# google/automl

Measured on NVIDIA H100. Metric: EfficientDet-D0 images/sec @ batch 32/GPU (640x640, forward + post-process), higher is better.
Workload: dtype f16 storage / f32 accumulate

## Files before the change

automl_b200/csrc/pointwise_tc.cu:

```cuda
#include <math_constants.h>

#include <type_traits>

#include "tc_common.cuh"

namespace edet {
namespace pwtc {

constexpr int BLOCK_M = 64;
constexpr int kMaxBlockN = 128;
template <int TEAMS>
struct Epi {
  static constexpr int kThreads = 128 * (1 + TEAMS);
};
constexpr int kStoreCols = 64;
constexpr int kSlabBytes = BLOCK_M * kStoreCols * 2;
constexpr int kMaxStages = 9;
constexpr int kRing = 4;
constexpr int kSmemLimit = 227 * 1024;
constexpr int kResidentWBytes = 108 * 1024;

struct Params {
  int batch, rows, k, nout, nout_pad8;
  int block_n, num_m_blocks, num_n_blocks, num_k_blocks, num_stages;
  int team_stages;
  int block_k;
  int a_stage_bytes, b_stage_bytes;
  int stage_bytes;
  int w_resident;
  int slab_sets;
  int slab_set_bytes;
  int desc_sbo;
  int desc_layout;
  int wbatch, ldr;
  int total_tiles;
  int bias_floats;
  const float* bias;
  const __half* residual;
  unsigned* sched;
  float* am_scores;
  int32_t* am_classes;
  int am_anchor_begin, am_total, am_num_anchors;
};
constexpr int EPI_STORE = 0, EPI_ARGMAX = 1;
constexpr int kArgmaxCols = 96;

struct TileCoord {
  int b, m_blk, n_blk;
};
constexpr int kMaxBiasSmem = 8192;

__device__ __forceinline__ TileCoord decode_tile(int t, const Params& p) {
  TileCoord c;
  c.n_blk = 0;
  if (p.num_n_blocks != 1) {
    c.n_blk = t % p.num_n_blocks;
    t /= p.num_n_blocks;
  }
  c.m_blk = t;
  c.b = 0;
  if (p.batch != 1) {
    c.m_blk = t % p.num_m_blocks;
    c.b = t / p.num_m_blocks;
  }
  return c;
}

__device__ __forceinline__ uint32_t argmax_pair_key(float2 s, uint32_t col) {
  const __half2 h = __hadd2(__floats2half2_rn(s.x, s.y), __float2half2_rn(0.f));
  const uint32_t hb = *reinterpret_cast<const uint32_t*>(&h);
  uint32_t sgn;
  asm("prmt.b32 %0, %1, %2, 0xBB99;" : "=r"(sgn) : "r"(hb), "r"(0u));
  const uint32_t ord = hb ^ (sgn | 0x80008000u);
  const uint32_t codes = ((0xFFFFu - (col + 1u)) << 16) | (0xFFFFu - col);
  uint32_t k0, k1;
  asm("prmt.b32 %0, %1, %2, 0x1054;" : "=r"(k0) : "r"(ord), "r"(codes));
  asm("prmt.b32 %0, %1, %2, 0x3276;" : "=r"(k1) : "r"(ord), "r"(codes));
  return max(k0, k1);
}

template <int ACT, bool HAS_RES, int TEAMS, int EPI>
__global__ void __launch_bounds__(Epi<TEAMS>::kThreads, 1)
pointwise_tc_kernel(const __grid_constant__ CUtensorMap map_a,
                    const __grid_constant__ CUtensorMap map_w,
                    const __grid_constant__ CUtensorMap map_o, const Params p) {
  pdl_launch_dependents();
  extern __shared__ __align__(1024) uint8_t smem_raw[];
  uint8_t* smem = reinterpret_cast<uint8_t*>(
      (reinterpret_cast<uintptr_t>(smem_raw) + 1023) & ~static_cast<uintptr_t>(1023));
  const int stage_bytes = p.stage_bytes;
  uint8_t* smem_w = smem + p.num_stages * stage_bytes;
  const int w_bytes = p.w_resident ? p.num_n_blocks * p.num_k_blocks * p.b_stage_bytes : 0;
  uint8_t* smem_store = smem_w + w_bytes;
  float* smem_bias = reinterpret_cast<float*>(smem_store + TEAMS * p.slab_sets * p.slab_set_bytes);
  uint64_t* bars = reinterpret_cast<uint64_t*>(smem_bias + p.bias_floats);
  uint64_t* full_bar = bars;
  uint64_t* empty_bar = bars + kMaxStages;
  uint64_t* ring_full = bars + 2 * kMaxStages;
  uint64_t* ring_empty = ring_full + kRing;
  uint64_t* w_full = ring_empty + kRing;
  volatile int4* tile_ring = reinterpret_cast<volatile int4*>(w_full + 2);

  const int warp = __shfl_sync(0xffffffffu, static_cast<int>(threadIdx.x >> 5), 0);
  const int lane = threadIdx.x & 31;

  if (threadIdx.x == 0) {
    for (int s = 0; s < p.num_stages; ++s) {
      mbar_init(smem_u32(&full_bar[s]), 1);
      mbar_init(smem_u32(&empty_bar[s]), 4);
    }
    for (int s = 0; s < kRing; ++s) {
      mbar_init(smem_u32(&ring_full[s]), 1);
      mbar_init(smem_u32(&ring_empty[s]), TEAMS);
    }
    mbar_init(smem_u32(&w_full[0]), 1);
    asm volatile("fence.mbarrier_init.release.cluster;" ::: "memory");
    asm volatile("prefetch.tensormap [%0];" ::"l"(reinterpret_cast<uint64_t>(&map_a)) : "memory");
    asm volatile("prefetch.tensormap [%0];" ::"l"(reinterpret_cast<uint64_t>(&map_w)) : "memory");
    asm volatile("prefetch.tensormap [%0];" ::"l"(reinterpret_cast<uint64_t>(&map_o)) : "memory");
  }
  for (int i = threadIdx.x; i < p.bias_floats; i += blockDim.x)
    smem_bias[i] = i < p.nout ? __ldg(p.bias + i) : 0.f;
  __syncthreads();
  pdl_wait_prior();

  if (warp == 0) {
    if (lane == 0) {
      const uint32_t w_box_bytes = static_cast<uint32_t>(p.block_n * p.block_k * 2);
      if (p.w_resident) {
        const uint32_t wb = smem_u32(&w_full[0]);
        mbar_expect_tx(wb, w_box_bytes * p.num_n_blocks * p.num_k_blocks);
        for (int nb = 0; nb < p.num_n_blocks; ++nb)
          for (int kb = 0; kb < p.num_k_blocks; ++kb)
            tma_load_3d(smem_u32(smem_w + (nb * p.num_k_blocks + kb) * p.b_stage_bytes), &map_w,
                        wb, kb * p.block_k, nb * p.block_n, 0);
      }
      int stage_of[TEAMS] = {}, phase_of[TEAMS] = {};
      const uint32_t tx_bytes =
          static_cast<uint32_t>(p.a_stage_bytes) + (p.w_resident ? 0u : w_box_bytes);
      bool exhausted = false;
      for (int i = 0;; ++i) {
        int t = p.total_tiles;
        if (i == 0) {
          t = blockIdx.x;
        } else if (!exhausted) {
          t = sched_next_tile(p.sched, p.total_tiles);
          exhausted = t >= p.total_tiles;
        }
        const int slot = i & (kRing - 1);
        mbar_wait(smem_u32(&ring_empty[slot]), (static_cast<uint32_t>(i / kRing) & 1u) ^ 1u);
        TileCoord tc;
        tc.b = tc.m_blk = tc.n_blk = 0;
        if (t < p.total_tiles) tc = decode_tile(t, p);
        const_cast<int4*>(tile_ring)[slot] = make_int4(t, tc.b, tc.m_blk, tc.n_blk);
        mbar_arrive(smem_u32(&ring_full[slot]));
        if (t >= p.total_tiles) break;
        const int wb = (p.wbatch > 1) ? tc.b : 0;
        const int team = i % TEAMS;
        int stage = stage_of[team];
        uint32_t phase = static_cast<uint32_t>(phase_of[team]);
        for (int kb = 0; kb < p.num_k_blocks; ++kb) {
          const int s = team * p.team_stages + stage;
          mbar_wait(smem_u32(&empty_bar[s]), phase ^ 1);
          const uint32_t fb = smem_u32(&full_bar[s]);
          mbar_expect_tx(fb, tx_bytes);
          uint8_t* sa = smem + s * stage_bytes;
          tma_load_3d(smem_u32(sa), &map_a, fb, kb * p.block_k, tc.m_blk * BLOCK_M, tc.b);
          if (!p.w_resident)
            tma_load_3d(smem_u32(sa + p.a_stage_bytes), &map_w, fb, kb * p.block_k,
                        tc.n_blk * p.block_n, wb);
          if (++stage == p.team_stages) {
            stage = 0;
            phase ^= 1;
          }
        }
        stage_of[team] = stage;
        phase_of[team] = static_cast<int>(phase);
      }
    }
  } else if (warp >= 4) {
    const int team = (warp >> 2) - 1;
    const int wtid = threadIdx.x & 127;
    const int r0 = 16 * (warp & 3) + (lane >> 2);
    const int cq = 2 * (lane & 3);
    uint8_t* team_slabs = smem_store + team * p.slab_sets * p.slab_set_bytes;
    if (p.w_resident) mbar_wait(smem_u32(&w_full[0]), 0);
    auto consume = [&](auto nt_const) {
    constexpr int NT = decltype(nt_const)::value;
    int my_tiles = 0;
    int stage = 0;
    uint32_t phase = 0;
    auto advance = [&]() {
      if (++stage == p.team_stages) {
        stage = 0;
        phase ^= 1;
      }
    };
    for (int iter = 0;; ++iter) {
      const int slot = iter & (kRing - 1);
      mbar_wait(smem_u32(&ring_full[slot]), static_cast<uint32_t>(iter / kRing) & 1u);
      int4 e = const_cast<const int4*>(tile_ring)[slot];
      e.x = __shfl_sync(0xffffffffu, e.x, 0);
      e.y = __shfl_sync(0xffffffffu, e.y, 0);
      e.z = __shfl_sync(0xffffffffu, e.z, 0);
      e.w = __shfl_sync(0xffffffffu, e.w, 0);
      named_sync(1 + team, 128);
      if (wtid == 0) mbar_arrive(smem_u32(&ring_empty[slot]));
      const int t = e.x;
      if (t >= p.total_tiles) break;
      if (iter % TEAMS != team) continue;
      TileCoord tc;
      tc.b = e.y;
      tc.m_blk = e.z;
      tc.n_blk = e.w;
      const int n0 = tc.n_blk * p.block_n;
      const int n_valid = min(p.block_n, ((p.nout - n0 + 15) >> 4) << 4);
      const int nt = n_valid >> 4;
      float acc[NT][8];
#pragma unroll
      for (int j = 0; j < NT; ++j)
#pragma unroll
        for (int q = 0; q < 8; ++q) acc[j][q] = 0.f;
      int prev_s = -1;
      for (int kb = 0; kb < p.num_k_blocks; ++kb) {
        const int s = team * p.team_stages + stage;
        mbar_wait(smem_u32(&full_bar[s]), phase);
        uint8_t* sa = smem + s * stage_bytes;
        uint8_t* sb = p.w_resident
                          ? smem_w + (tc.n_blk * p.num_k_blocks + kb) * p.b_stage_bytes
                          : sa + p.a_stage_bytes;
        const uint64_t da = make_smem_desc(smem_u32(sa), p.desc_sbo, p.desc_layout);
        const uint64_t db = make_smem_desc(smem_u32(sb), p.desc_sbo, p.desc_layout);
        const int k_rem = p.k - kb * p.block_k;
        const int ksteps = k_rem >= p.block_k ? p.block_k / MMA_K : (k_rem + MMA_K - 1) / MMA_K;
        wg_fence();
        wg_mma_kblock_wide<NT>(acc, da, db, ksteps, kb == 0);
        wg_commit();
        wg_wait<1>();
        if (prev_s >= 0) {
          __syncwarp();
          if (lane == 0) mbar_arrive(smem_u32(&empty_bar[prev_s]));
        }
        prev_s = s;
        advance();
      }
      wg_wait<0>();
      __syncwarp();
      if (lane == 0) mbar_arrive(smem_u32(&empty_bar[prev_s]));
      wg_fence_acc<NT>(acc);
      const int row0 = tc.m_blk * BLOCK_M + r0;
      if constexpr (EPI == EPI_ARGMAX) {
        const float* bias = smem_bias + tc.n_blk * kArgmaxCols;
        uint32_t best[2] = {0u, 0u};
#pragma unroll
        for (int j = 0; j < kArgmaxCols / 16; ++j) {
#pragma unroll
          for (int h = 0; h < 2; ++h) {
            const int col = 16 * j + 8 * h + cq;
            const float2 b = *reinterpret_cast<const float2*>(bias + col);
#pragma unroll
            for (int r = 0; r < 2; ++r) {
              const float2 s = fadd2_rn(make_float2(acc[j][4 * h + 2 * r], acc[j][4 * h + 2 * r + 1]), b);
              best[r] = max(best[r], argmax_pair_key(s, static_cast<uint32_t>(col)));
            }
          }
        }
#pragma unroll
        for (int r = 0; r < 2; ++r) {
          best[r] = max(best[r], __shfl_xor_sync(0xffffffffu, best[r], 1));
          best[r] = max(best[r], __shfl_xor_sync(0xffffffffu, best[r], 2));
          const uint32_t ord_best = best[r] >> 16;
          const unsigned short hbits = static_cast<unsigned short>(
              (ord_best & 0x8000u) ? (ord_best ^ 0x8000u) : (~ord_best & 0xFFFFu));
          const float bv = __half2float(__ushort_as_half(hbits));
          const int best_c = static_cast<int>(0xFFFFu - (best[r] & 0xFFFFu));
          const int row = row0 + 8 * r;
          if ((lane & 3) == 0 && row < p.rows) {
            const size_t o = static_cast<size_t>(tc.b) * p.am_total + p.am_anchor_begin +
                             static_cast<size_t>(row) * p.am_num_anchors + tc.n_blk;
            p.am_scores[o] = __fdiv_rn(1.0f, __fadd_rn(1.0f, expf(-bv)));
            p.am_classes[o] = best_c;
          }
        }
      } else {
        const bool ok[2] = {row0 < p.rows, row0 + 8 < p.rows};
        const __half* res_row[2] = {nullptr, nullptr};
        if (HAS_RES) {
#pragma unroll
          for (int r = 0; r < 2; ++r)
            res_row[r] = p.residual +
                         (static_cast<size_t>(tc.b) * p.rows + (ok[r] ? row0 + 8 * r : 0)) * p.ldr;
        }
        uint8_t* my_slabs = team_slabs + (my_tiles % p.slab_sets) * p.slab_set_bytes;
        ++my_tiles;
        if (wtid == 0) {
          if (p.slab_sets == 2)
            tma_store_wait_read<1>();
          else
            tma_store_wait_read<0>();
        }
        named_sync(1 + team, 128);
#pragma unroll
        for (int j = 0; j < NT; ++j) {
          if (j < nt) {
            const int colt = 16 * j + cq;
            const float2 b_lo = *reinterpret_cast<const float2*>(smem_bias + n0 + colt);
            const float2 b_hi = *reinterpret_cast<const float2*>(smem_bias + n0 + colt + 8);
            uint8_t* slab = my_slabs + (colt >> 6) * kSlabBytes;
            const int piece = (colt & 63) >> 3;
#pragma unroll
            for (int r = 0; r < 2; ++r) {
              float2 lo = fadd2_rn(make_float2(acc[j][2 * r], acc[j][2 * r + 1]), b_lo);
              float2 hi = fadd2_rn(make_float2(acc[j][4 + 2 * r], acc[j][4 + 2 * r + 1]), b_hi);
              apply_act4<ACT>(lo, hi);
              if (HAS_RES && ok[r]) {
                const int col = n0 + colt;
                if (col < p.nout)
                  lo = fadd2_rn(lo, __half22float2(*reinterpret_cast<const __half2*>(res_row[r] + col)));
                if (col + 8 < p.nout)
                  hi = fadd2_rn(hi, __half22float2(*reinterpret_cast<const __half2*>(res_row[r] + col + 8)));
              }
              const int row = r0 + 8 * r;
              uint8_t* rb = slab + row * 128 + cq * 2;
              *reinterpret_cast<__half2*>(rb + ((piece ^ (row & 7)) << 4)) = __floats2half2_rn(lo.x, lo.y);
              *reinterpret_cast<__half2*>(rb + (((piece + 1) ^ (row & 7)) << 4)) = __floats2half2_rn(hi.x, hi.y);
            }
          }
        }
        fence_proxy_async_smem();
        named_sync(1 + team, 128);
        if (wtid == 0) {
          for (int c = 0; c * kStoreCols < n_valid; ++c)
            tma_store_3d(&map_o, smem_u32(my_slabs + c * kSlabBytes), n0 + c * kStoreCols,
                         tc.m_blk * BLOCK_M, tc.b);
          tma_store_commit();
        }
      }
    }
    };
    if constexpr (EPI == EPI_ARGMAX) {
      consume(std::integral_constant<int, kArgmaxCols / 16>{});
    } else {
      switch (p.block_n >> 5) {
        case 1: consume(std::integral_constant<int, 2>{}); break;
        case 2: consume(std::integral_constant<int, 4>{}); break;
        case 3: consume(std::integral_constant<int, 6>{}); break;
        default: consume(std::integral_constant<int, 8>{}); break;
      }
    }
    if (wtid == 0) tma_store_wait_all();
  }
}

static int pick_block_n(int nout) {
  if (nout <= kMaxBlockN) return ((nout + 31) / 32) * 32;
  return kMaxBlockN;
}

template <int ACT, bool HAS_RES, int TEAMS, int EPI = EPI_STORE>
static int launch(const CUtensorMap& ma, const CUtensorMap& mw, const CUtensorMap& mo,
                  const Params& p, int grid, int smem_bytes, cudaStream_t stream) {
  auto kern = pointwise_tc_kernel<ACT, HAS_RES, TEAMS, EPI>;
  static int configured[kMaxDevices];
  if (int rc = ensure_dynamic_smem(kern, kSmemLimit, configured)) return rc;
  EDET_CHECK_CUDA(launch_pdl(kern, dim3(grid), dim3(Epi<TEAMS>::kThreads), smem_bytes, stream, ma,
                             mw, mo, p));
  return EDET_OK;
}

int run(const __half* a, int lda, const __half* wt, int wbatch, const float* bias,
        const __half* residual, int ldr, __half* out, int ldo, int batch, int rows, int k, int nout,
        int act, cudaStream_t stream, const ArgmaxArgs* am) {
  Params p;
  p.am_scores = nullptr; p.am_classes = nullptr;
  p.am_anchor_begin = p.am_total = p.am_num_anchors = 0;
  if (am) {
    EDET_CHECK_ARG(nout == am->num_anchors * kArgmaxCols && !residual && act == EDET_ACT_NONE,
                   "class_argmax: nout must be num_anchors * %d", kArgmaxCols);
    p.am_scores = am->scores; p.am_classes = am->classes;
    p.am_anchor_begin = am->anchor_begin; p.am_total = am->total_anchors;
    p.am_num_anchors = am->num_anchors;
  }
  p.batch = batch;
  p.rows = rows;
  p.k = k;
  p.nout = nout;
  p.nout_pad8 = nout & ~7;
  const int opt_teams = option_pw_teams();
  const int teams = opt_teams ? opt_teams : 2;
  p.block_n = am ? kArgmaxCols : pick_block_n(nout);
  p.num_m_blocks = ceil_div(rows, BLOCK_M);
  p.num_n_blocks = ceil_div(nout, p.block_n);
  p.wbatch = wbatch;
  p.ldr = ldr;
  p.bias = bias;
  p.residual = residual;
  p.total_tiles = batch * p.num_m_blocks * p.num_n_blocks;
  p.sched = next_sched_slot();
  if (!p.sched) return EDET_ERR_CUDA;

  const int bias_cols = p.num_n_blocks * p.block_n;
  EDET_CHECK_ARG(bias_cols <= kMaxBiasSmem, "pointwise_tc: nout %d too wide", nout);
  p.bias_floats = bias_cols;
  p.block_k = k <= 16 ? 16 : (k <= 32 ? 32 : 64);
  p.a_stage_bytes = BLOCK_M * p.block_k * 2;
  p.b_stage_bytes = ((p.block_n * p.block_k * 2 + 1023) / 1024) * 1024;
  p.num_k_blocks = ceil_div(k, p.block_k);
  const int w_bytes = p.num_n_blocks * p.num_k_blocks * p.b_stage_bytes;
  p.w_resident = wbatch == 1 && w_bytes <= kResidentWBytes;
  p.stage_bytes = p.a_stage_bytes + (p.w_resident ? 0 : p.b_stage_bytes);
  p.slab_set_bytes = am ? 0 : ceil_div(p.block_n, kStoreCols) * kSlabBytes;
  const int opt_kb = option_pw_smem_kb();
  const int limit = opt_kb ? opt_kb * 1024 : kSmemLimit;
  auto fixed_bytes = [&](int sets) {
    return (p.w_resident ? w_bytes : 0) + teams * sets * p.slab_set_bytes + p.bias_floats * 4 +
           (2 * kMaxStages + 2 * kRing + 2) * 8 + 16 * kRing;
  };
  p.slab_sets = (limit - 1024 - fixed_bytes(2)) / p.stage_bytes >= 3 * teams ? 2 : 1;
  const int fixed = fixed_bytes(p.slab_sets);
  int stages = (limit - 1024 - fixed) / p.stage_bytes;
  if (stages > kMaxStages) stages = kMaxStages;
  p.team_stages = stages / teams;
  EDET_CHECK_ARG(p.team_stages >= 2, "pointwise_tc: block_n %d leaves <2 pipeline stages per consumer",
                 p.block_n);
  stages = p.team_stages * teams;
  p.num_stages = stages;
  p.desc_layout = desc_layout_for(p.block_k);
  p.desc_sbo = 8 * p.block_k * 2;
  const int smem_bytes = 1024 + stages * p.stage_bytes + fixed;

  CUtensorMap ma, mw, mo;
  int rc;
  if ((rc = make_map(&ma, a, k, rows, batch, lda, static_cast<uint64_t>(rows) * lda, BLOCK_M,
                     p.block_k)))
    return rc;
  if ((rc = make_map(&mw, wt, k, nout, wbatch, k, static_cast<uint64_t>(nout) * k, p.block_n,
                     p.block_k)))
    return rc;
  if (am) {
    mo = mw;
  } else if ((rc = make_map(&mo, out, nout, rows, batch, ldo, static_cast<uint64_t>(rows) * ldo,
                            BLOCK_M, kStoreCols))) {
    return rc;
  }

  const int sm_count = device_sm_count();
  if (!sm_count) return EDET_ERR_CUDA;
  int grid = sm_count - option_persist_slack();
  if (grid < 1) grid = 1;
  if (p.total_tiles < grid) grid = p.total_tiles;
  const bool has_res = residual != nullptr;
  if (am) return launch<EDET_ACT_NONE, false, 2, EPI_ARGMAX>(ma, mw, mo, p, grid, smem_bytes, stream);

#define EDET_PW_CASE(A)                                                                       \
  if (teams == 3)                                                                             \
    return has_res ? launch<A, true, 3>(ma, mw, mo, p, grid, smem_bytes, stream)              \
                   : launch<A, false, 3>(ma, mw, mo, p, grid, smem_bytes, stream);            \
  return has_res ? launch<A, true, 2>(ma, mw, mo, p, grid, smem_bytes, stream)                \
                 : launch<A, false, 2>(ma, mw, mo, p, grid, smem_bytes, stream)
  switch (act) {
    case EDET_ACT_NONE: EDET_PW_CASE(EDET_ACT_NONE);
    case EDET_ACT_SWISH: EDET_PW_CASE(EDET_ACT_SWISH);
    case EDET_ACT_RELU: EDET_PW_CASE(EDET_ACT_RELU);
    case EDET_ACT_RELU6: EDET_PW_CASE(EDET_ACT_RELU6);
    case EDET_ACT_HSWISH: EDET_PW_CASE(EDET_ACT_HSWISH);
    case EDET_ACT_SIGMOID: EDET_PW_CASE(EDET_ACT_SIGMOID);
    default:
      set_error("pointwise_tc: bad activation %d", act);
      return EDET_ERR_INVALID;
  }
#undef EDET_PW_CASE
}

}
}
```

automl_b200/csrc/tc_common.cuh:

```cuda
#pragma once
#include <cuda.h>

#include "common.cuh"

namespace edet {
namespace pwtc {

constexpr int MMA_K = 16;

struct ArgmaxArgs {
  float* scores;
  int32_t* classes;
  int anchor_begin, total_anchors, num_anchors;
};
int run(const __half* a, int lda, const __half* wt, int wbatch, const float* bias,
        const __half* residual, int ldr, __half* out, int ldo, int batch, int rows, int k, int nout,
        int act, cudaStream_t stream, const ArgmaxArgs* am = nullptr);

__device__ __forceinline__ uint32_t smem_u32(const void* p) {
  return static_cast<uint32_t>(__cvta_generic_to_shared(p));
}
__device__ __forceinline__ void mbar_init(uint32_t bar, uint32_t count) {
  asm volatile("mbarrier.init.shared::cta.b64 [%0], %1;" ::"r"(bar), "r"(count));
}
__device__ __forceinline__ void mbar_expect_tx(uint32_t bar, uint32_t bytes) {
  asm volatile("mbarrier.arrive.expect_tx.shared::cta.b64 _, [%0], %1;" ::"r"(bar), "r"(bytes)
               : "memory");
}
__device__ __forceinline__ void mbar_arrive(uint32_t bar) {
  asm volatile("mbarrier.arrive.shared::cta.b64 _, [%0];" ::"r"(bar) : "memory");
}
__device__ __forceinline__ void mbar_wait(uint32_t bar, uint32_t parity) {
  asm volatile(
      "{\n\t"
      ".reg .pred p;\n\t"
      "WAIT_LOOP:\n\t"
      "mbarrier.try_wait.parity.shared::cta.b64 p, [%0], %1;\n\t"
      "@p bra DONE;\n\t"
      "bra WAIT_LOOP;\n\t"
      "DONE:\n\t"
      "}" ::"r"(bar),
      "r"(parity)
      : "memory");
}
__device__ __forceinline__ void tma_load_3d(uint32_t dst, const CUtensorMap* map, uint32_t bar,
                                            int c0, int c1, int c2) {
  asm volatile(
      "cp.async.bulk.tensor.3d.shared::cluster.global.mbarrier::complete_tx::bytes "
      "[%0], [%1, {%3, %4, %5}], [%2];" ::"r"(dst),
      "l"(reinterpret_cast<uint64_t>(map)), "r"(bar), "r"(c0), "r"(c1), "r"(c2)
      : "memory");
}
__device__ __forceinline__ void tma_store_3d(const CUtensorMap* map, uint32_t src, int c0, int c1,
                                             int c2) {
  asm volatile(
      "cp.async.bulk.tensor.3d.global.shared::cta.bulk_group [%0, {%2, %3, %4}], [%1];" ::"l"(
          reinterpret_cast<uint64_t>(map)),
      "r"(src), "r"(c0), "r"(c1), "r"(c2)
      : "memory");
}
__device__ __forceinline__ void tma_store_4d(const CUtensorMap* map, uint32_t src, int c0, int c1,
                                             int c2, int c3) {
  asm volatile(
      "cp.async.bulk.tensor.4d.global.shared::cta.bulk_group [%0, {%2, %3, %4, %5}], [%1];" ::"l"(
          reinterpret_cast<uint64_t>(map)),
      "r"(src), "r"(c0), "r"(c1), "r"(c2), "r"(c3)
      : "memory");
}
__device__ __forceinline__ void tma_store_commit() {
  asm volatile("cp.async.bulk.commit_group;" ::: "memory");
}
template <int N>
__device__ __forceinline__ void tma_store_wait_read() {
  asm volatile("cp.async.bulk.wait_group.read %0;" ::"n"(N) : "memory");
}
__device__ __forceinline__ void tma_store_wait_all() {
  asm volatile("cp.async.bulk.wait_group 0;" ::: "memory");
}
__device__ __forceinline__ void fence_proxy_async_smem() {
  asm volatile("fence.proxy.async.shared::cta;" ::: "memory");
}
__device__ __forceinline__ void wg_fence() { asm volatile("wgmma.fence.sync.aligned;" ::: "memory"); }
__device__ __forceinline__ void wg_commit() {
  asm volatile("wgmma.commit_group.sync.aligned;" ::: "memory");
}
template <int N>
__device__ __forceinline__ void wg_wait() {
  asm volatile("wgmma.wait_group.sync.aligned %0;" ::"n"(N) : "memory");
}
__device__ __forceinline__ void wg_mma_m64n16(float* d, uint64_t desc_a, uint64_t desc_b,
                                              uint32_t accumulate) {
  asm volatile(
      "{\n\t"
      ".reg .pred p;\n\t"
      "setp.ne.b32 p, %10, 0;\n\t"
      "wgmma.mma_async.sync.aligned.m64n16k16.f32.f16.f16 "
      "{%0, %1, %2, %3, %4, %5, %6, %7}, %8, %9, p, 1, 1, 0, 0;\n\t"
      "}"
      : "+f"(d[0]), "+f"(d[1]), "+f"(d[2]), "+f"(d[3]), "+f"(d[4]), "+f"(d[5]), "+f"(d[6]),
        "+f"(d[7])
      : "l"(desc_a), "l"(desc_b), "r"(accumulate)
      : "memory");
}
template <int NT>
__device__ __forceinline__ void wg_fence_acc(float (&acc)[NT][8]) {
#pragma unroll
  for (int j = 0; j < NT; ++j)
#pragma unroll
    for (int e = 0; e < 8; ++e) asm volatile("" : "+f"(acc[j][e])::"memory");
}
template <int NT>
__device__ __forceinline__ void wg_mma_kblock(float (&acc)[NT][8], uint64_t desc_a,
                                              uint64_t desc_b, int b_chunk, int nt, int ksteps,
                                              bool first) {
  for (int ks = 0; ks < ksteps; ++ks) {
#pragma unroll
    for (int j = 0; j < NT; ++j) {
      if (j < nt)
        wg_mma_m64n16(acc[j], desc_a + static_cast<uint64_t>(ks * 2),
                      desc_b + static_cast<uint64_t>(j * b_chunk + ks * 2),
                      (first && ks == 0) ? 0u : 1u);
    }
  }
}
__device__ __forceinline__ void wg_mma_m64n32(float* d, uint64_t desc_a, uint64_t desc_b,
                                              uint32_t accumulate) {
  asm volatile(
      "{\n\t"
      ".reg .pred p;\n\t"
      "setp.ne.b32 p, %18, 0;\n\t"
      "wgmma.mma_async.sync.aligned.m64n32k16.f32.f16.f16 "
      "{%0, %1, %2, %3, %4, %5, %6, %7, %8, %9, %10, %11, %12, %13, %14, %15}, "
      "%16, %17, p, 1, 1, 0, 0;\n\t"
      "}"
      : "+f"(d[0]), "+f"(d[1]), "+f"(d[2]), "+f"(d[3]), "+f"(d[4]), "+f"(d[5]), "+f"(d[6]), "+f"(d[7]),
        "+f"(d[8]), "+f"(d[9]), "+f"(d[10]), "+f"(d[11]), "+f"(d[12]), "+f"(d[13]), "+f"(d[14]), "+f"(d[15])
      : "l"(desc_a), "l"(desc_b), "r"(accumulate)
      : "memory");
}
__device__ __forceinline__ void wg_mma_m64n64(float* d, uint64_t desc_a, uint64_t desc_b,
                                              uint32_t accumulate) {
  asm volatile(
      "{\n\t"
      ".reg .pred p;\n\t"
      "setp.ne.b32 p, %34, 0;\n\t"
      "wgmma.mma_async.sync.aligned.m64n64k16.f32.f16.f16 "
      "{%0, %1, %2, %3, %4, %5, %6, %7, %8, %9, %10, %11, %12, %13, %14, %15,"
      " %16, %17, %18, %19, %20, %21, %22, %23, %24, %25, %26, %27, %28, %29, %30, %31}, "
      "%32, %33, p, 1, 1, 0, 0;\n\t"
      "}"
      : "+f"(d[0]), "+f"(d[1]), "+f"(d[2]), "+f"(d[3]), "+f"(d[4]), "+f"(d[5]), "+f"(d[6]), "+f"(d[7]),
        "+f"(d[8]), "+f"(d[9]), "+f"(d[10]), "+f"(d[11]), "+f"(d[12]), "+f"(d[13]), "+f"(d[14]), "+f"(d[15]),
        "+f"(d[16]), "+f"(d[17]), "+f"(d[18]), "+f"(d[19]), "+f"(d[20]), "+f"(d[21]), "+f"(d[22]), "+f"(d[23]),
        "+f"(d[24]), "+f"(d[25]), "+f"(d[26]), "+f"(d[27]), "+f"(d[28]), "+f"(d[29]), "+f"(d[30]), "+f"(d[31])
      : "l"(desc_a), "l"(desc_b), "r"(accumulate)
      : "memory");
}
__device__ __forceinline__ void wg_mma_m64n96(float* d, uint64_t desc_a, uint64_t desc_b,
                                              uint32_t accumulate) {
  asm volatile(
      "{\n\t"
      ".reg .pred p;\n\t"
      "setp.ne.b32 p, %50, 0;\n\t"
      "wgmma.mma_async.sync.aligned.m64n96k16.f32.f16.f16 "
      "{%0, %1, %2, %3, %4, %5, %6, %7, %8, %9, %10, %11, %12, %13, %14, %15,"
      " %16, %17, %18, %19, %20, %21, %22, %23, %24, %25, %26, %27, %28, %29, %30, %31,"
      " %32, %33, %34, %35, %36, %37, %38, %39, %40, %41, %42, %43, %44, %45, %46, %47}, "
      "%48, %49, p, 1, 1, 0, 0;\n\t"
      "}"
      : "+f"(d[0]), "+f"(d[1]), "+f"(d[2]), "+f"(d[3]), "+f"(d[4]), "+f"(d[5]), "+f"(d[6]), "+f"(d[7]),
        "+f"(d[8]), "+f"(d[9]), "+f"(d[10]), "+f"(d[11]), "+f"(d[12]), "+f"(d[13]), "+f"(d[14]), "+f"(d[15]),
        "+f"(d[16]), "+f"(d[17]), "+f"(d[18]), "+f"(d[19]), "+f"(d[20]), "+f"(d[21]), "+f"(d[22]), "+f"(d[23]),
        "+f"(d[24]), "+f"(d[25]), "+f"(d[26]), "+f"(d[27]), "+f"(d[28]), "+f"(d[29]), "+f"(d[30]), "+f"(d[31]),
        "+f"(d[32]), "+f"(d[33]), "+f"(d[34]), "+f"(d[35]), "+f"(d[36]), "+f"(d[37]), "+f"(d[38]), "+f"(d[39]),
        "+f"(d[40]), "+f"(d[41]), "+f"(d[42]), "+f"(d[43]), "+f"(d[44]), "+f"(d[45]), "+f"(d[46]), "+f"(d[47])
      : "l"(desc_a), "l"(desc_b), "r"(accumulate)
      : "memory");
}
__device__ __forceinline__ void wg_mma_m64n128(float* d, uint64_t desc_a, uint64_t desc_b,
                                              uint32_t accumulate) {
  asm volatile(
      "{\n\t"
      ".reg .pred p;\n\t"
      "setp.ne.b32 p, %66, 0;\n\t"
      "wgmma.mma_async.sync.aligned.m64n128k16.f32.f16.f16 "
      "{%0, %1, %2, %3, %4, %5, %6, %7, %8, %9, %10, %11, %12, %13, %14, %15,"
      " %16, %17, %18, %19, %20, %21, %22, %23, %24, %25, %26, %27, %28, %29, %30, %31,"
      " %32, %33, %34, %35, %36, %37, %38, %39, %40, %41, %42, %43, %44, %45, %46, %47,"
      " %48, %49, %50, %51, %52, %53, %54, %55, %56, %57, %58, %59, %60, %61, %62, %63}, "
      "%64, %65, p, 1, 1, 0, 0;\n\t"
      "}"
      : "+f"(d[0]), "+f"(d[1]), "+f"(d[2]), "+f"(d[3]), "+f"(d[4]), "+f"(d[5]), "+f"(d[6]), "+f"(d[7]),
        "+f"(d[8]), "+f"(d[9]), "+f"(d[10]), "+f"(d[11]), "+f"(d[12]), "+f"(d[13]), "+f"(d[14]), "+f"(d[15]),
        "+f"(d[16]), "+f"(d[17]), "+f"(d[18]), "+f"(d[19]), "+f"(d[20]), "+f"(d[21]), "+f"(d[22]), "+f"(d[23]),
        "+f"(d[24]), "+f"(d[25]), "+f"(d[26]), "+f"(d[27]), "+f"(d[28]), "+f"(d[29]), "+f"(d[30]), "+f"(d[31]),
        "+f"(d[32]), "+f"(d[33]), "+f"(d[34]), "+f"(d[35]), "+f"(d[36]), "+f"(d[37]), "+f"(d[38]), "+f"(d[39]),
        "+f"(d[40]), "+f"(d[41]), "+f"(d[42]), "+f"(d[43]), "+f"(d[44]), "+f"(d[45]), "+f"(d[46]), "+f"(d[47]),
        "+f"(d[48]), "+f"(d[49]), "+f"(d[50]), "+f"(d[51]), "+f"(d[52]), "+f"(d[53]), "+f"(d[54]), "+f"(d[55]),
        "+f"(d[56]), "+f"(d[57]), "+f"(d[58]), "+f"(d[59]), "+f"(d[60]), "+f"(d[61]), "+f"(d[62]), "+f"(d[63])
      : "l"(desc_a), "l"(desc_b), "r"(accumulate)
      : "memory");
}
template <int NT>
__device__ __forceinline__ void wg_mma_kblock_wide(float (&acc)[NT][8], uint64_t desc_a,
                                                   uint64_t desc_b, int ksteps, bool first) {
  static_assert(NT == 2 || NT == 4 || NT == 6 || NT == 8, "wide wgmma: N = 32, 64, 96 or 128");
  float* d = &acc[0][0];
  for (int ks = 0; ks < ksteps; ++ks) {
    const uint64_t a = desc_a + static_cast<uint64_t>(ks * 2);
    const uint64_t b = desc_b + static_cast<uint64_t>(ks * 2);
    const uint32_t accumulate = (first && ks == 0) ? 0u : 1u;
    if constexpr (NT == 2) wg_mma_m64n32(d, a, b, accumulate);
    if constexpr (NT == 4) wg_mma_m64n64(d, a, b, accumulate);
    if constexpr (NT == 6) wg_mma_m64n96(d, a, b, accumulate);
    if constexpr (NT == 8) wg_mma_m64n128(d, a, b, accumulate);
  }
}
__device__ __forceinline__ void named_sync(int id, int threads) {
  asm volatile("bar.sync %0, %1;" ::"r"(id), "r"(threads) : "memory");
}

__device__ __forceinline__ uint64_t make_smem_desc(uint32_t saddr, int sbo, int layout) {
  uint64_t d = 0;
  d |= static_cast<uint64_t>((saddr & 0x3FFFF) >> 4);
  d |= static_cast<uint64_t>(1) << 16;
  d |= static_cast<uint64_t>(sbo >> 4) << 32;
  d |= static_cast<uint64_t>(layout) << 62;
  return d;
}
inline int desc_layout_for(int block_k) { return block_k == 64 ? 1 : (block_k == 32 ? 2 : 3); }


__device__ __forceinline__ void tma_load_4d(uint32_t dst, const CUtensorMap* map, uint32_t bar,
                                            int c0, int c1, int c2, int c3) {
  asm volatile(
      "cp.async.bulk.tensor.4d.shared::cluster.global.mbarrier::complete_tx::bytes "
      "[%0], [%1, {%3, %4, %5, %6}], [%2];" ::"r"(dst),
      "l"(reinterpret_cast<uint64_t>(map)), "r"(bar), "r"(c0), "r"(c1), "r"(c2), "r"(c3)
      : "memory");
}

__device__ __forceinline__ int sched_next_tile(unsigned* sched, int total_tiles) {
  const int t = static_cast<int>(gridDim.x + atomicAdd(&sched[0], 1u));
  if (t >= total_tiles) {
    __threadfence();
    if (atomicAdd(&sched[1], 1u) == gridDim.x - 1) {
      sched[0] = 0u;
      sched[1] = 0u;
      __threadfence();
    }
  }
  return t;
}
constexpr int kSchedSlots = 4096;
typedef CUresult (*EncodeTiledFn)(CUtensorMap*, CUtensorMapDataType, cuuint32_t, void*,
                                  const cuuint64_t*, const cuuint64_t*, const cuuint32_t*,
                                  const cuuint32_t*, CUtensorMapInterleave, CUtensorMapSwizzle,
                                  CUtensorMapL2promotion, CUtensorMapFloatOOBfill);

inline EncodeTiledFn get_encode_fn() {
  static EncodeTiledFn fn = nullptr;
  if (fn) return fn;
  void* sym = nullptr;
  cudaDriverEntryPointQueryResult qres;
  if (cudaGetDriverEntryPoint("cuTensorMapEncodeTiled", &sym, cudaEnableDefault, &qres) !=
          cudaSuccess ||
      qres != cudaDriverEntryPointSuccess || sym == nullptr) {
    return nullptr;
  }
  fn = reinterpret_cast<EncodeTiledFn>(sym);
  return fn;
}

unsigned* next_sched_slot();

inline int make_map(CUtensorMap* map, const void* ptr, uint64_t d0, uint64_t d1, uint64_t d2,
                    uint64_t stride1_elems, uint64_t stride2_elems, uint32_t box1,
                    uint32_t box0 = 64) {
  EncodeTiledFn fn = get_encode_fn();
  if (!fn) {
    set_error("cuTensorMapEncodeTiled entry point not available");
    return EDET_ERR_CUDA;
  }
  cuuint64_t dims[3] = {d0, d1, d2};
  cuuint64_t strides[2] = {stride1_elems * 2, stride2_elems * 2};
  cuuint32_t box[3] = {box0, box1, 1};
  const CUtensorMapSwizzle swz = box0 == 64 ? CU_TENSOR_MAP_SWIZZLE_128B
                                 : box0 == 32 ? CU_TENSOR_MAP_SWIZZLE_64B
                                              : CU_TENSOR_MAP_SWIZZLE_32B;
  cuuint32_t estr[3] = {1, 1, 1};
  CUresult r = fn(map, CU_TENSOR_MAP_DATA_TYPE_FLOAT16, 3, const_cast<void*>(ptr), dims, strides,
                  box, estr, CU_TENSOR_MAP_INTERLEAVE_NONE, swz,
                  CU_TENSOR_MAP_L2_PROMOTION_L2_256B, CU_TENSOR_MAP_FLOAT_OOB_FILL_NONE);
  if (r != CUDA_SUCCESS) {
    set_error("cuTensorMapEncodeTiled failed (%d) dims=[%llu,%llu,%llu] strides=[%llu,%llu] box1=%u",
              static_cast<int>(r), (unsigned long long)d0, (unsigned long long)d1,
              (unsigned long long)d2, (unsigned long long)strides[0],
              (unsigned long long)strides[1], box1);
    return EDET_ERR_CUDA;
  }
  return EDET_OK;
}


inline int make_map4(CUtensorMap* map, const void* ptr, uint64_t d0, uint64_t d1, uint64_t d2,
                     uint64_t d3, uint32_t box0, uint32_t box1, uint32_t box2, bool swizzle = true) {
  EncodeTiledFn fn = get_encode_fn();
  if (!fn) {
    set_error("cuTensorMapEncodeTiled entry point not available");
    return EDET_ERR_CUDA;
  }
  cuuint64_t dims[4] = {d0, d1, d2, d3};
  cuuint64_t strides[3] = {d0 * 2, d0 * d1 * 2, d0 * d1 * d2 * 2};
  cuuint32_t box[4] = {box0, box1, box2, 1};
  cuuint32_t estr[4] = {1, 1, 1, 1};
  const CUtensorMapSwizzle swz = !swizzle      ? CU_TENSOR_MAP_SWIZZLE_NONE
                                 : box0 == 64 ? CU_TENSOR_MAP_SWIZZLE_128B
                                 : box0 == 32 ? CU_TENSOR_MAP_SWIZZLE_64B
                                              : CU_TENSOR_MAP_SWIZZLE_32B;
  CUresult r = fn(map, CU_TENSOR_MAP_DATA_TYPE_FLOAT16, 4, const_cast<void*>(ptr), dims, strides,
                  box, estr, CU_TENSOR_MAP_INTERLEAVE_NONE, swz, CU_TENSOR_MAP_L2_PROMOTION_L2_256B,
                  CU_TENSOR_MAP_FLOAT_OOB_FILL_NONE);
  if (r != CUDA_SUCCESS) {
    set_error("cuTensorMapEncodeTiled(4d) failed (%d) dims=[%llu,%llu,%llu,%llu] box=[%u,%u,%u]",
              static_cast<int>(r), (unsigned long long)d0, (unsigned long long)d1,
              (unsigned long long)d2, (unsigned long long)d3, box0, box1, box2);
    return EDET_ERR_CUDA;
  }
  return EDET_OK;
}

inline int make_map4_strided(CUtensorMap* map, const void* ptr, uint64_t d0, uint64_t d1,
                             uint64_t d2, uint64_t d3, uint64_t s1, uint64_t s2, uint64_t s3,
                             uint32_t box0, uint32_t box1, uint32_t box2) {
  EncodeTiledFn fn = get_encode_fn();
  if (!fn) {
    set_error("cuTensorMapEncodeTiled entry point not available");
    return EDET_ERR_CUDA;
  }
  cuuint64_t dims[4] = {d0, d1, d2, d3};
  cuuint64_t strides[3] = {s1 * 2, s2 * 2, s3 * 2};
  cuuint32_t box[4] = {box0, box1, box2, 1};
  cuuint32_t estr[4] = {1, 1, 1, 1};
  const CUtensorMapSwizzle swz = box0 == 64 ? CU_TENSOR_MAP_SWIZZLE_128B
                                 : box0 == 32 ? CU_TENSOR_MAP_SWIZZLE_64B
                                              : CU_TENSOR_MAP_SWIZZLE_32B;
  CUresult r = fn(map, CU_TENSOR_MAP_DATA_TYPE_FLOAT16, 4, const_cast<void*>(ptr), dims, strides,
                  box, estr, CU_TENSOR_MAP_INTERLEAVE_NONE, swz, CU_TENSOR_MAP_L2_PROMOTION_L2_256B,
                  CU_TENSOR_MAP_FLOAT_OOB_FILL_NONE);
  if (r != CUDA_SUCCESS) {
    set_error("cuTensorMapEncodeTiled(4d strided) failed (%d) dims=[%llu,%llu,%llu,%llu] "
              "strides=[%llu,%llu,%llu] box=[%u,%u,%u]", static_cast<int>(r),
              (unsigned long long)d0, (unsigned long long)d1, (unsigned long long)d2,
              (unsigned long long)d3, (unsigned long long)strides[0],
              (unsigned long long)strides[1], (unsigned long long)strides[2], box0, box1, box2);
    return EDET_ERR_CUDA;
  }
  return EDET_OK;
}

}
}
```

Baseline: 4871.

## Schedule multi-m-block work units and reuse resident A tile across n-blocks

The persistent pointwise GEMM now hands out work units of several consecutive m-blocks instead of single tiles. When weights are resident and K fits in one block, one unit covers every n-block, so the A tile is loaded once and reused. The scheduler claims the next unit one step ahead so atomic latency overlaps loading, and pipeline depth is sized by a bytes-in-flight target rather than a fixed stage cap. The cost is coarser load balancing and possible tail imbalance from larger units, plus more complex stage and phase bookkeeping across n-blocks.

```diff
diff --git a/automl_b200/csrc/pointwise_tc.cu b/automl_b200/csrc/pointwise_tc.cu
--- a/automl_b200/csrc/pointwise_tc.cu
+++ b/automl_b200/csrc/pointwise_tc.cu
@@ -1,5 +1,6 @@
 #include <math_constants.h>
 
+#include <algorithm>
 #include <type_traits>
 
 #include "tc_common.cuh"
@@ -15,10 +16,14 @@
 };
 constexpr int kStoreCols = 64;
 constexpr int kSlabBytes = BLOCK_M * kStoreCols * 2;
-constexpr int kMaxStages = 9;
+constexpr int kTeamInFlightBytes = 32 * 1024;
+constexpr int kMinTeamStages = 4;
+constexpr int kMaxStages = 3 * 16;
 constexpr int kRing = 4;
 constexpr int kSmemLimit = 227 * 1024;
 constexpr int kResidentWBytes = 108 * 1024;
+constexpr int kUnitsPerCta = 8;
+constexpr int kMaxUnitBytes = 128 * 1024;
 
 struct Params {
   int batch, rows, k, nout, nout_pad8;
@@ -33,7 +38,9 @@
   int desc_sbo;
   int desc_layout;
   int wbatch, ldr;
-  int total_tiles;
+  int unit_m, units_per_image;
+  int hold_a;
+  int total_units;
   int bias_floats;
   const float* bias;
   const __half* residual;
@@ -50,19 +57,20 @@
 };
 constexpr int kMaxBiasSmem = 8192;
 
-__device__ __forceinline__ TileCoord decode_tile(int t, const Params& p) {
+__device__ __forceinline__ TileCoord decode_unit(int u, const Params& p) {
   TileCoord c;
   c.n_blk = 0;
-  if (p.num_n_blocks != 1) {
-    c.n_blk = t % p.num_n_blocks;
-    t /= p.num_n_blocks;
-  }
-  c.m_blk = t;
+  if (p.num_n_blocks != 1 && !p.hold_a) {
+    c.n_blk = u % p.num_n_blocks;
+    u /= p.num_n_blocks;
+  }
+  c.m_blk = u;
   c.b = 0;
   if (p.batch != 1) {
-    c.m_blk = t % p.num_m_blocks;
-    c.b = t / p.num_m_blocks;
-  }
+    c.m_blk = u % p.units_per_image;
+    c.b = u / p.units_per_image;
+  }
+  c.m_blk *= p.unit_m;
   return c;
 }
 
@@ -138,44 +146,43 @@
       int stage_of[TEAMS] = {}, phase_of[TEAMS] = {};
       const uint32_t tx_bytes =
           static_cast<uint32_t>(p.a_stage_bytes) + (p.w_resident ? 0u : w_box_bytes);
-      bool exhausted = false;
+      int u = blockIdx.x;
       for (int i = 0;; ++i) {
-        int t = p.total_tiles;
-        if (i == 0) {
-          t = blockIdx.x;
-        } else if (!exhausted) {
-          t = sched_next_tile(p.sched, p.total_tiles);
-          exhausted = t >= p.total_tiles;
-        }
+        const int next = u < p.total_units ? sched_claim(p.sched) : p.total_units;
         const int slot = i & (kRing - 1);
         mbar_wait(smem_u32(&ring_empty[slot]), (static_cast<uint32_t>(i / kRing) & 1u) ^ 1u);
         TileCoord tc;
         tc.b = tc.m_blk = tc.n_blk = 0;
-        if (t < p.total_tiles) tc = decode_tile(t, p);
-        const_cast<int4*>(tile_ring)[slot] = make_int4(t, tc.b, tc.m_blk, tc.n_blk);
+        if (u < p.total_units) tc = decode_unit(u, p);
+        const_cast<int4*>(tile_ring)[slot] = make_int4(u, tc.b, tc.m_blk, tc.n_blk);
         mbar_arrive(smem_u32(&ring_full[slot]));
-        if (t >= p.total_tiles) break;
+        if (u >= p.total_units) break;
         const int wb = (p.wbatch > 1) ? tc.b : 0;
         const int team = i % TEAMS;
         int stage = stage_of[team];
         uint32_t phase = static_cast<uint32_t>(phase_of[team]);
-        for (int kb = 0; kb < p.num_k_blocks; ++kb) {
-          const int s = team * p.team_stages + stage;
-          mbar_wait(smem_u32(&empty_bar[s]), phase ^ 1);
-          const uint32_t fb = smem_u32(&full_bar[s]);
-          mbar_expect_tx(fb, tx_bytes);
-          uint8_t* sa = smem + s * stage_bytes;
-          tma_load_3d(smem_u32(sa), &map_a, fb, kb * p.block_k, tc.m_blk * BLOCK_M, tc.b);
-          if (!p.w_resident)
-            tma_load_3d(smem_u32(sa + p.a_stage_bytes), &map_w, fb, kb * p.block_k,
-                        tc.n_blk * p.block_n, wb);
-          if (++stage == p.team_stages) {
-            stage = 0;
-            phase ^= 1;
+        const int m_end = min(tc.m_blk + p.unit_m, p.num_m_blocks);
+        for (int m_blk = tc.m_blk; m_blk < m_end; ++m_blk) {
+          for (int kb = 0; kb < p.num_k_blocks; ++kb) {
+            const int s = team * p.team_stages + stage;
+            mbar_wait(smem_u32(&empty_bar[s]), phase ^ 1);
+            const uint32_t fb = smem_u32(&full_bar[s]);
+            mbar_expect_tx(fb, tx_bytes);
+            uint8_t* sa = smem + s * stage_bytes;
+            tma_load_3d(smem_u32(sa), &map_a, fb, kb * p.block_k, m_blk * BLOCK_M, tc.b);
+            if (!p.w_resident)
+              tma_load_3d(smem_u32(sa + p.a_stage_bytes), &map_w, fb, kb * p.block_k,
+                          tc.n_blk * p.block_n, wb);
+            if (++stage == p.team_stages) {
+              stage = 0;
+              phase ^= 1;
+            }
           }
         }
         stage_of[team] = stage;
         phase_of[team] = static_cast<int>(phase);
+        u = next;
+        if (u >= p.total_units) sched_retire(p.sched);
       }
     }
   } else if (warp >= 4) {
@@ -206,134 +213,140 @@
       e.w = __shfl_sync(0xffffffffu, e.w, 0);
       named_sync(1 + team, 128);
       if (wtid == 0) mbar_arrive(smem_u32(&ring_empty[slot]));
-      const int t = e.x;
-      if (t >= p.total_tiles) break;
+      if (e.x >= p.total_units) break;
       if (iter % TEAMS != team) continue;
+      const int m_end = min(e.z + p.unit_m, p.num_m_blocks);
+      const int n_end = p.hold_a ? p.num_n_blocks : e.w + 1;
       TileCoord tc;
       tc.b = e.y;
-      tc.m_blk = e.z;
-      tc.n_blk = e.w;
-      const int n0 = tc.n_blk * p.block_n;
-      const int n_valid = min(p.block_n, ((p.nout - n0 + 15) >> 4) << 4);
-      const int nt = n_valid >> 4;
-      float acc[NT][8];
-#pragma unroll
-      for (int j = 0; j < NT; ++j)
-#pragma unroll
-        for (int q = 0; q < 8; ++q) acc[j][q] = 0.f;
-      int prev_s = -1;
-      for (int kb = 0; kb < p.num_k_blocks; ++kb) {
-        const int s = team * p.team_stages + stage;
-        mbar_wait(smem_u32(&full_bar[s]), phase);
-        uint8_t* sa = smem + s * stage_bytes;
-        uint8_t* sb = p.w_resident
-                          ? smem_w + (tc.n_blk * p.num_k_blocks + kb) * p.b_stage_bytes
-                          : sa + p.a_stage_bytes;
-        const uint64_t da = make_smem_desc(smem_u32(sa), p.desc_sbo, p.desc_layout);
-        const uint64_t db = make_smem_desc(smem_u32(sb), p.desc_sbo, p.desc_layout);
-        const int k_rem = p.k - kb * p.block_k;
-        const int ksteps = k_rem >= p.block_k ? p.block_k / MMA_K : (k_rem + MMA_K - 1) / MMA_K;
-        wg_fence();
-        wg_mma_kblock_wide<NT>(acc, da, db, ksteps, kb == 0);
-        wg_commit();
-        wg_wait<1>();
-        if (prev_s >= 0) {
-          __syncwarp();
-          if (lane == 0) mbar_arrive(smem_u32(&empty_bar[prev_s]));
-        }
-        prev_s = s;
-        advance();
-      }
-      wg_wait<0>();
-      __syncwarp();
-      if (lane == 0) mbar_arrive(smem_u32(&empty_bar[prev_s]));
-      wg_fence_acc<NT>(acc);
-      const int row0 = tc.m_blk * BLOCK_M + r0;
-      if constexpr (EPI == EPI_ARGMAX) {
-        const float* bias = smem_bias + tc.n_blk * kArgmaxCols;
-        uint32_t best[2] = {0u, 0u};
-#pragma unroll
-        for (int j = 0; j < kArgmaxCols / 16; ++j) {
-#pragma unroll
-          for (int h = 0; h < 2; ++h) {
-            const int col = 16 * j + 8 * h + cq;
-            const float2 b = *reinterpret_cast<const float2*>(bias + col);
+      for (tc.m_blk = e.z; tc.m_blk < m_end; ++tc.m_blk) {
+        for (tc.n_blk = e.w; tc.n_blk < n_end; ++tc.n_blk) {
+          const bool last_n = tc.n_blk + 1 == n_end;
+          const int n0 = tc.n_blk * p.block_n;
+          const int n_valid = min(p.block_n, ((p.nout - n0 + 15) >> 4) << 4);
+          const int nt = n_valid >> 4;
+          float acc[NT][8];
+#pragma unroll
+          for (int j = 0; j < NT; ++j)
+#pragma unroll
+            for (int q = 0; q < 8; ++q) acc[j][q] = 0.f;
+          int prev_s = -1;
+          for (int kb = 0; kb < p.num_k_blocks; ++kb) {
+            const int s = team * p.team_stages + stage;
+            if (tc.n_blk == e.w) mbar_wait(smem_u32(&full_bar[s]), phase);
+            uint8_t* sa = smem + s * stage_bytes;
+            uint8_t* sb = p.w_resident
+                              ? smem_w + (tc.n_blk * p.num_k_blocks + kb) * p.b_stage_bytes
+                              : sa + p.a_stage_bytes;
+            const uint64_t da = make_smem_desc(smem_u32(sa), p.desc_sbo, p.desc_layout);
+            const uint64_t db = make_smem_desc(smem_u32(sb), p.desc_sbo, p.desc_layout);
+            const int k_rem = p.k - kb * p.block_k;
+            const int ksteps = k_rem >= p.block_k ? p.block_k / MMA_K : (k_rem + MMA_K - 1) / MMA_K;
+            wg_fence();
+            wg_mma_kblock_wide<NT>(acc, da, db, ksteps, kb == 0);
+            wg_commit();
+            wg_wait<1>();
+            if (prev_s >= 0) {
+              __syncwarp();
+              if (lane == 0) mbar_arrive(smem_u32(&empty_bar[prev_s]));
+            }
+            prev_s = s;
+            if (last_n) advance();
+          }
+          wg_wait<0>();
+          if (last_n) {
+            __syncwarp();
+            if (lane == 0) mbar_arrive(smem_u32(&empty_bar[prev_s]));
+          }
+          wg_fence_acc<NT>(acc);
+          const int row0 = tc.m_blk * BLOCK_M + r0;
+          if constexpr (EPI == EPI_ARGMAX) {
+            const float* bias = smem_bias + tc.n_blk * kArgmaxCols;
+            uint32_t best[2] = {0u, 0u};
+#pragma unroll
+            for (int j = 0; j < kArgmaxCols / 16; ++j) {
+#pragma unroll
+              for (int h = 0; h < 2; ++h) {
+                const int col = 16 * j + 8 * h + cq;
+                const float2 b = *reinterpret_cast<const float2*>(bias + col);
+#pragma unroll
+                for (int r = 0; r < 2; ++r) {
+                  const float2 s = fadd2_rn(make_float2(acc[j][4 * h + 2 * r], acc[j][4 * h + 2 * r + 1]), b);
+                  best[r] = max(best[r], argmax_pair_key(s, static_cast<uint32_t>(col)));
+                }
+              }
+            }
 #pragma unroll
             for (int r = 0; r < 2; ++r) {
-              const float2 s = fadd2_rn(make_float2(acc[j][4 * h + 2 * r], acc[j][4 * h + 2 * r + 1]), b);
-              best[r] = max(best[r], argmax_pair_key(s, static_cast<uint32_t>(col)));
+              best[r] = max(best[r], __shfl_xor_sync(0xffffffffu, best[r], 1));
+              best[r] = max(best[r], __shfl_xor_sync(0xffffffffu, best[r], 2));
+              const uint32_t ord_best = best[r] >> 16;
+              const unsigned short hbits = static_cast<unsigned short>(
+                  (ord_best & 0x8000u) ? (ord_best ^ 0x8000u) : (~ord_best & 0xFFFFu));
+              const float bv = __half2float(__ushort_as_half(hbits));
+              const int best_c = static_cast<int>(0xFFFFu - (best[r] & 0xFFFFu));
+              const int row = row0 + 8 * r;
+              if ((lane & 3) == 0 && row < p.rows) {
+                const size_t o = static_cast<size_t>(tc.b) * p.am_total + p.am_anchor_begin +
+                                 static_cast<size_t>(row) * p.am_num_anchors + tc.n_blk;
+                p.am_scores[o] = __fdiv_rn(1.0f, __fadd_rn(1.0f, expf(-bv)));
+                p.am_classes[o] = best_c;
+              }
+            }
+          } else {
+            const bool ok[2] = {row0 < p.rows, row0 + 8 < p.rows};
+            const __half* res_row[2] = {nullptr, nullptr};
+            if (HAS_RES) {
+#pragma unroll
+              for (int r = 0; r < 2; ++r)
+                res_row[r] = p.residual +
+                             (static_cast<size_t>(tc.b) * p.rows + (ok[r] ? row0 + 8 * r : 0)) * p.ldr;
+            }
+            uint8_t* my_slabs = team_slabs + (my_tiles % p.slab_sets) * p.slab_set_bytes;
+            ++my_tiles;
+            if (wtid == 0) {
+              if (p.slab_sets == 2)
+                tma_store_wait_read<1>();
+              else
+                tma_store_wait_read<0>();
+            }
+            named_sync(1 + team, 128);
+#pragma unroll
+            for (int j = 0; j < NT; ++j) {
+              if (j < nt) {
+                const int colt = 16 * j + cq;
+                const float2 b_lo = *reinterpret_cast<const float2*>(smem_bias + n0 + colt);
+                const float2 b_hi = *reinterpret_cast<const float2*>(smem_bias + n0 + colt + 8);
+                uint8_t* slab = my_slabs + (colt >> 6) * kSlabBytes;
+                const int piece = (colt & 63) >> 3;
+#pragma unroll
+                for (int r = 0; r < 2; ++r) {
+                  float2 lo = fadd2_rn(make_float2(acc[j][2 * r], acc[j][2 * r + 1]), b_lo);
+                  float2 hi = fadd2_rn(make_float2(acc[j][4 + 2 * r], acc[j][4 + 2 * r + 1]), b_hi);
+                  apply_act4<ACT>(lo, hi);
+                  if (HAS_RES && ok[r]) {
+                    const int col = n0 + colt;
+                    if (col < p.nout)
+                      lo = fadd2_rn(lo, __half22float2(*reinterpret_cast<const __half2*>(res_row[r] + col)));
+                    if (col + 8 < p.nout)
+                      hi = fadd2_rn(hi, __half22float2(*reinterpret_cast<const __half2*>(res_row[r] + col + 8)));
+                  }
+                  const int row = r0 + 8 * r;
+                  uint8_t* rb = slab + row * 128 + cq * 2;
+                  *reinterpret_cast<__half2*>(rb + ((piece ^ (row & 7)) << 4)) = __floats2half2_rn(lo.x, lo.y);
+                  *reinterpret_cast<__half2*>(rb + (((piece + 1) ^ (row & 7)) << 4)) = __floats2half2_rn(hi.x, hi.y);
+                }
+              }
+            }
+            fence_proxy_async_smem();
+            named_sync(1 + team, 128);
+            if (wtid == 0) {
+              for (int c = 0; c * kStoreCols < n_valid; ++c)
+                tma_store_3d(&map_o, smem_u32(my_slabs + c * kSlabBytes), n0 + c * kStoreCols,
+                             tc.m_blk * BLOCK_M, tc.b);
+              tma_store_commit();
             }
           }
-        }
-#pragma unroll
-        for (int r = 0; r < 2; ++r) {
-          best[r] = max(best[r], __shfl_xor_sync(0xffffffffu, best[r], 1));
-          best[r] = max(best[r], __shfl_xor_sync(0xffffffffu, best[r], 2));
-          const uint32_t ord_best = best[r] >> 16;
-          const unsigned short hbits = static_cast<unsigned short>(
-              (ord_best & 0x8000u) ? (ord_best ^ 0x8000u) : (~ord_best & 0xFFFFu));
-          const float bv = __half2float(__ushort_as_half(hbits));
-          const int best_c = static_cast<int>(0xFFFFu - (best[r] & 0xFFFFu));
-          const int row = row0 + 8 * r;
-          if ((lane & 3) == 0 && row < p.rows) {
-            const size_t o = static_cast<size_t>(tc.b) * p.am_total + p.am_anchor_begin +
-                             static_cast<size_t>(row) * p.am_num_anchors + tc.n_blk;
-            p.am_scores[o] = __fdiv_rn(1.0f, __fadd_rn(1.0f, expf(-bv)));
-            p.am_classes[o] = best_c;
-          }
-        }
-      } else {
-        const bool ok[2] = {row0 < p.rows, row0 + 8 < p.rows};
-        const __half* res_row[2] = {nullptr, nullptr};
-        if (HAS_RES) {
-#pragma unroll
-          for (int r = 0; r < 2; ++r)
-            res_row[r] = p.residual +
-                         (static_cast<size_t>(tc.b) * p.rows + (ok[r] ? row0 + 8 * r : 0)) * p.ldr;
-        }
-        uint8_t* my_slabs = team_slabs + (my_tiles % p.slab_sets) * p.slab_set_bytes;
-        ++my_tiles;
-        if (wtid == 0) {
-          if (p.slab_sets == 2)
-            tma_store_wait_read<1>();
-          else
-            tma_store_wait_read<0>();
-        }
-        named_sync(1 + team, 128);
-#pragma unroll
-        for (int j = 0; j < NT; ++j) {
-          if (j < nt) {
-            const int colt = 16 * j + cq;
-            const float2 b_lo = *reinterpret_cast<const float2*>(smem_bias + n0 + colt);
-            const float2 b_hi = *reinterpret_cast<const float2*>(smem_bias + n0 + colt + 8);
-            uint8_t* slab = my_slabs + (colt >> 6) * kSlabBytes;
-            const int piece = (colt & 63) >> 3;
-#pragma unroll
-            for (int r = 0; r < 2; ++r) {
-              float2 lo = fadd2_rn(make_float2(acc[j][2 * r], acc[j][2 * r + 1]), b_lo);
-              float2 hi = fadd2_rn(make_float2(acc[j][4 + 2 * r], acc[j][4 + 2 * r + 1]), b_hi);
-              apply_act4<ACT>(lo, hi);
-              if (HAS_RES && ok[r]) {
-                const int col = n0 + colt;
-                if (col < p.nout)
-                  lo = fadd2_rn(lo, __half22float2(*reinterpret_cast<const __half2*>(res_row[r] + col)));
-                if (col + 8 < p.nout)
-                  hi = fadd2_rn(hi, __half22float2(*reinterpret_cast<const __half2*>(res_row[r] + col + 8)));
-              }
-              const int row = r0 + 8 * r;
-              uint8_t* rb = slab + row * 128 + cq * 2;
-              *reinterpret_cast<__half2*>(rb + ((piece ^ (row & 7)) << 4)) = __floats2half2_rn(lo.x, lo.y);
-              *reinterpret_cast<__half2*>(rb + (((piece + 1) ^ (row & 7)) << 4)) = __floats2half2_rn(hi.x, hi.y);
-            }
-          }
-        }
-        fence_proxy_async_smem();
-        named_sync(1 + team, 128);
-        if (wtid == 0) {
-          for (int c = 0; c * kStoreCols < n_valid; ++c)
-            tma_store_3d(&map_o, smem_u32(my_slabs + c * kSlabBytes), n0 + c * kStoreCols,
-                         tc.m_blk * BLOCK_M, tc.b);
-          tma_store_commit();
         }
       }
     }
@@ -395,7 +408,6 @@
   p.ldr = ldr;
   p.bias = bias;
   p.residual = residual;
-  p.total_tiles = batch * p.num_m_blocks * p.num_n_blocks;
   p.sched = next_sched_slot();
   if (!p.sched) return EDET_ERR_CUDA;
 
@@ -409,6 +421,7 @@
   const int w_bytes = p.num_n_blocks * p.num_k_blocks * p.b_stage_bytes;
   p.w_resident = wbatch == 1 && w_bytes <= kResidentWBytes;
   p.stage_bytes = p.a_stage_bytes + (p.w_resident ? 0 : p.b_stage_bytes);
+
   p.slab_set_bytes = am ? 0 : ceil_div(p.block_n, kStoreCols) * kSlabBytes;
   const int opt_kb = option_pw_smem_kb();
   const int limit = opt_kb ? opt_kb * 1024 : kSmemLimit;
@@ -418,12 +431,35 @@
   };
   p.slab_sets = (limit - 1024 - fixed_bytes(2)) / p.stage_bytes >= 3 * teams ? 2 : 1;
   const int fixed = fixed_bytes(p.slab_sets);
-  int stages = (limit - 1024 - fixed) / p.stage_bytes;
-  if (stages > kMaxStages) stages = kMaxStages;
-  p.team_stages = stages / teams;
-  EDET_CHECK_ARG(p.team_stages >= 2, "pointwise_tc: block_n %d leaves <2 pipeline stages per consumer",
+  const int max_team_stages =
+      std::min((limit - 1024 - fixed) / p.stage_bytes, kMaxStages) / teams;
+  EDET_CHECK_ARG(max_team_stages >= 2, "pointwise_tc: block_n %d leaves <2 pipeline stages per consumer",
                  p.block_n);
-  stages = p.team_stages * teams;
+
+  const int sm_count = device_sm_count();
+  if (!sm_count) return EDET_ERR_CUDA;
+  int grid = sm_count - option_persist_slack();
+  if (grid < 1) grid = 1;
+  p.hold_a = p.w_resident && p.num_n_blocks > 1 && p.num_k_blocks == 1 &&
+             batch * p.num_m_blocks >= grid;
+  const int unit_n_blocks = p.hold_a ? p.num_n_blocks : 1;
+  const int m_block_bytes =
+      p.num_k_blocks * p.stage_bytes + unit_n_blocks * BLOCK_M * p.block_n * 2;
+  auto units_for = [&](int g) {
+    return batch * ceil_div(p.num_m_blocks, g) * (p.hold_a ? 1 : p.num_n_blocks);
+  };
+  p.unit_m = 8;
+  while (p.unit_m > 1 && (units_for(p.unit_m) < kUnitsPerCta * grid ||
+                          p.unit_m * m_block_bytes > kMaxUnitBytes ||
+                          p.unit_m * p.num_k_blocks > max_team_stages))
+    p.unit_m >>= 1;
+  p.units_per_image = ceil_div(p.num_m_blocks, p.unit_m);
+  p.total_units = units_for(p.unit_m);
+  if (p.total_units < grid) grid = p.total_units;
+  p.team_stages = std::min(max_team_stages,
+                           std::max({kMinTeamStages, ceil_div(kTeamInFlightBytes, p.stage_bytes),
+                                     p.unit_m * p.num_k_blocks}));
+  const int stages = p.team_stages * teams;
   p.num_stages = stages;
   p.desc_layout = desc_layout_for(p.block_k);
   p.desc_sbo = 8 * p.block_k * 2;
@@ -444,11 +480,6 @@
     return rc;
   }
 
-  const int sm_count = device_sm_count();
-  if (!sm_count) return EDET_ERR_CUDA;
-  int grid = sm_count - option_persist_slack();
-  if (grid < 1) grid = 1;
-  if (p.total_tiles < grid) grid = p.total_tiles;
   const bool has_res = residual != nullptr;
   if (am) return launch<EDET_ACT_NONE, false, 2, EPI_ARGMAX>(ma, mw, mo, p, grid, smem_bytes, stream);
 
diff --git a/automl_b200/csrc/tc_common.cuh b/automl_b200/csrc/tc_common.cuh
--- a/automl_b200/csrc/tc_common.cuh
+++ b/automl_b200/csrc/tc_common.cuh
@@ -240,16 +240,20 @@
       : "memory");
 }
 
+__device__ __forceinline__ int sched_claim(unsigned* sched) {
+  return static_cast<int>(gridDim.x + atomicAdd(&sched[0], 1u));
+}
+__device__ __forceinline__ void sched_retire(unsigned* sched) {
+  __threadfence();
+  if (atomicAdd(&sched[1], 1u) == gridDim.x - 1) {
+    sched[0] = 0u;
+    sched[1] = 0u;
+    __threadfence();
+  }
+}
 __device__ __forceinline__ int sched_next_tile(unsigned* sched, int total_tiles) {
-  const int t = static_cast<int>(gridDim.x + atomicAdd(&sched[0], 1u));
-  if (t >= total_tiles) {
-    __threadfence();
-    if (atomicAdd(&sched[1], 1u) == gridDim.x - 1) {
-      sched[0] = 0u;
-      sched[1] = 0u;
-      __threadfence();
-    }
-  }
+  const int t = sched_claim(sched);
+  if (t >= total_tiles) sched_retire(sched);
   return t;
 }
 constexpr int kSchedSlots = 4096;
```

Result: faster. 5175 (median of 6 runs) (+6.2%).
